# mohammadasim98/mv-ldm

Hardware: AMD Instinct MI355X
Metric: denoised views/sec @ 256x256, 4 views, 50 DDIM steps (higher is better)
Workload: dtype bf16

## Files before the change

### mv_ldm_amd/_lib.py

```python
from __future__ import annotations

import ctypes as C
from pathlib import Path

LIB_PATH = Path(__file__).resolve().parent / "csrc" / "libmvldm_hip.so"

ABI_VERSION = 7
F32, BF16, F16 = 0, 1, 2
EPI_NONE, EPI_SILU, EPI_GEGLU, EPI_GELU = 0, 1, 2, 3
RAYS_RAW, RAYS_POSITIONAL, RAYS_SRT = 0, 1, 2
ELT_COPY, ELT_SILU, ELT_GELU = 0, 1, 2
NORM_BWD_STORE = 0x100
GN_MAX_CHUNKS = 32

(OP_IGEMM, OP_GROUPNORM, OP_LAYERNORM, OP_ATTENTION, OP_TIMESTEP_EMBED, OP_ELTWISE, OP_DDIM_STEP, OP_DDIM_ADVANCE,
 OP_NCHW_TO_NHWC, OP_NHWC_TO_NCHW, OP_MEMCPY, OP_RAY_ENCODE, OP_POSTERIOR_SAMPLE,
 OP_WGRAD, OP_ATTENTION_BWD, OP_GROUPNORM_BWD, OP_LAYERNORM_BWD, OP_COLSUM, OP_TRAIN_ELTWISE, OP_POOL2X2, OP_ZERO_INSERT,
 OP_ADD_NOISE, OP_MSE_LOSS, OP_FILL_ZERO, OP_PAR_BEGIN, OP_PAR_NEXT, OP_PAR_END, OP_GATHER_ROWS, OP_ATTN_MERGE) = range(1, 30)
TE_SILU_BWD, TE_ADD, TE_GEGLU_FWD, TE_GEGLU_BWD, TE_GELU_BWD = 0, 1, 2, 3, 4

vp, i32, f32, sz = C.c_void_p, C.c_int32, C.c_float, C.c_size_t


class IgemmDesc(C.Structure):
    _fields_ = [("src0", vp), ("src1", vp), ("weight", vp), ("bias", vp), ("row_bias", vp), ("residual", vp),
                ("dst", vp), ("workspace", vp),
                ("c0", i32), ("c1", i32),
                ("n_img", i32), ("h_in", i32), ("w_in", i32), ("h_out", i32), ("w_out", i32),
                ("ksize", i32), ("stride", i32), ("pad", i32), ("upsample", i32),
                ("n_out", i32), ("n_pad", i32), ("k_pad", i32),
                ("row_bias_ld", i32), ("epilogue", i32), ("act_dtype", i32), ("dst_dtype", i32),
                ("splitk", i32), ("tile", i32), ("k_order", i32), ("dst_ld", i32), ("out_scale", f32), ("workspace_bytes", sz)]


class _GroupNorm(C.Structure):
    _fields_ = [("x", vp), ("x1", vp), ("y", vp), ("gamma", vp), ("beta", vp), ("stats_ws", vp),
                ("n_img", i32), ("hw", i32), ("c0", i32), ("c1", i32), ("groups", i32), ("silu", i32), ("dtype", i32),
                ("eps", f32), ("stats_out", vp)]


class _LayerNorm(C.Structure):
    _fields_ = [("x", vp), ("y", vp), ("gamma", vp), ("beta", vp), ("rows", i32), ("c", i32), ("dtype", i32), ("eps", f32)]


class _Attention(C.Structure):
    _fields_ = [("q", vp), ("k", vp), ("v", vp), ("out", vp), ("seg", vp),
                ("ld_q", i32), ("ld_k", i32), ("ld_v", i32), ("ld_o", i32), ("heads", i32), ("head_dim", i32),
                ("n_seg", i32), ("max_q_len", i32), ("dtype", i32), ("scale", f32), ("lse", vp), ("lse_ld", i32)]


class _Temb(C.Structure):
    _fields_ = [("timesteps", vp), ("freqs", vp), ("out", vp), ("n", i32), ("dim", i32), ("flip", i32), ("dst_dtype", i32)]


class _Eltwise(C.Structure):
    _fields_ = [("x", vp), ("y", vp), ("n", sz), ("op", i32), ("src_dtype", i32), ("dst_dtype", i32)]


class _Ddim(C.Structure):
    _fields_ = [("eps", vp), ("x_t", vp), ("x_next", vp), ("cond_img", vp), ("uncond_img", vp), ("coef", vp),
                ("step_ptr", vp), ("unet_in", vp),
                ("n_tgt", i32), ("hw", i32), ("c", i32), ("unet_in_c", i32), ("unet_in_dtype", i32), ("cfg_scale", f32),
                ("n_steps", i32), ("clip_range", f32)]


class _Advance(C.Structure):
    _fields_ = [("step_ptr", vp), ("t_table", vp), ("timesteps", vp), ("tgt_rows", vp), ("n_steps", i32), ("n_rows", i32)]


class _Layout(C.Structure):
    _fields_ = [("src", vp), ("dst", vp), ("n_img", i32), ("c", i32), ("hw", i32), ("other_c", i32),
                ("other_c_off", i32), ("dtype", i32), ("clamp01", i32), ("scale", f32), ("shift", f32), ("img_map", vp)]


class _Rays(C.Structure):
    _fields_ = [("extrinsics", vp), ("intrinsics", vp), ("out_nchw", vp), ("out_nhwc", vp), ("img_map", vp),
                ("n_cam", i32), ("h", i32), ("w", i32), ("nhwc_c", i32), ("nhwc_c_off", i32), ("nhwc_dtype", i32),
                ("mode", i32), ("n_origin_octaves", i32), ("n_dir_octaves", i32), ("plucker", i32)]


class _Posterior(C.Structure):
    _fields_ = [("moments", vp), ("noise", vp), ("out", vp), ("n", i32), ("c", i32), ("hw", i32), ("scale", f32)]


class _Memcpy(C.Structure):
    _fields_ = [("src", vp), ("dst", vp), ("bytes", sz)]


class _AttnMerge(C.Structure):
    _fields_ = [("oa", vp), ("ob", vp), ("out", vp), ("lse_a", vp), ("lse_b", vp), ("a_img", vp), ("b_img", vp), ("out_img", vp),
                ("n_img", i32), ("tokens", i32), ("heads", i32), ("head_dim", i32), ("ld_a", i32), ("ld_b", i32), ("ld_o", i32),
                ("lse_ld_a", i32), ("lse_ld_b", i32), ("dtype", i32)]


class _Gather(C.Structure):
    _fields_ = [("src", vp), ("dst", vp), ("src_index", vp), ("dst_index", vp), ("row_bytes", sz), ("n_rows", i32)]


class PackJob(C.Structure):
    _fields_ = [("src", vp), ("dst", vp), ("n_out", i32), ("c_in", i32), ("ksize", i32), ("c_pad", i32), ("n_pad", i32), ("k_pad", i32),
                ("geglu", i32), ("k_order", i32), ("transpose", i32), ("c_off", i32), ("n_rows", i32), ("kind", i32), ("blocks", i32),
                ("block0", i32)]


class WgradDesc(C.Structure):
    _fields_ = [("src0", vp), ("src1", vp), ("dy", vp), ("grad", vp), ("workspace", vp), ("workspace_bytes", sz),
                ("c0", i32), ("c1", i32), ("c_in", i32),
                ("n_img", i32), ("h_in", i32), ("w_in", i32), ("h_out", i32), ("w_out", i32),
                ("ksize", i32), ("stride", i32), ("pad", i32), ("upsample", i32),
                ("n_out", i32), ("dy_ld", i32), ("act_dtype", i32), ("accumulate", i32)]


class AttnBwdDesc(C.Structure):
    _fields_ = [("q", vp), ("k", vp), ("v", vp), ("out", vp), ("dout", vp), ("dq", vp), ("dk", vp), ("dv", vp),
                ("lse", vp), ("delta", vp), ("seg", vp),
                ("ld_q", i32), ("ld_k", i32), ("ld_v", i32), ("ld_o", i32), ("ld_do", i32), ("ld_dq", i32), ("ld_dk", i32), ("ld_dv", i32),
                ("heads", i32), ("head_dim", i32), ("n_seg", i32), ("max_q_len", i32), ("max_kv_len", i32), ("total_q_rows", i32),
                ("stat_ld", i32), ("dtype", i32), ("scale", f32)]


class _GroupNormBwd(C.Structure):
    _fields_ = [("x0", vp), ("x1", vp), ("dy", vp), ("dx0", vp), ("dx1", vp), ("gamma", vp), ("beta", vp), ("stats", vp),
                ("dgamma", vp), ("dbeta", vp), ("workspace", vp), ("workspace_bytes", sz),
                ("n_img", i32), ("hw", i32), ("c0", i32), ("c1", i32), ("groups", i32), ("silu", i32), ("dtype", i32)]


class _LayerNormBwd(C.Structure):
    _fields_ = [("x", vp), ("dy", vp), ("dx", vp), ("gamma", vp), ("dgamma", vp), ("dbeta", vp), ("workspace", vp),
                ("workspace_bytes", sz), ("rows", i32), ("c", i32), ("dtype", i32), ("eps", f32)]


class _Colsum(C.Structure):
    _fields_ = [("x", vp), ("dst", vp), ("workspace", vp), ("workspace_bytes", sz),
                ("n_seg", i32), ("rows_per_seg", i32), ("n", i32), ("ld", i32), ("ld_dst", i32), ("per_seg", i32),
                ("accumulate", i32), ("dtype", i32)]


class _TrainEltwise(C.Structure):
    _fields_ = [("a", vp), ("b", vp), ("out", vp), ("rows", sz), ("op", i32), ("d", i32), ("a_dtype", i32), ("dtype", i32)]


class _Resample(C.Structure):
    _fields_ = [("src", vp), ("dst", vp), ("n_img", i32), ("h", i32), ("w", i32), ("c", i32), ("dtype", i32)]


class _AddNoise(C.Structure):
    _fields_ = [("x0", vp), ("noise", vp), ("coef", vp), ("dst", vp), ("img_map", vp),
                ("n", i32), ("c", i32), ("hw", i32), ("dst_c", i32), ("dst_c_off", i32), ("dst_dtype", i32)]


class _Mse(C.Structure):
    _fields_ = [("pred", vp), ("noise", vp), ("tgt_img", vp), ("loss", vp), ("dpred", vp), ("workspace", vp),
                ("n_tgt", i32), ("hw", i32), ("c", i32), ("accumulate", i32), ("dpred_c", i32), ("dpred_dtype", i32),
                ("loss_scale", f32), ("grad_scale", f32), ("amp_scale", vp)]


class AmpState(C.Structure):
    _fields_ = [("scale", f32), ("growth_tracker", i32), ("adam_step", i32), ("found_inf", i32), ("skipped", i32), ("reserved", i32 * 3)]


class _Fill(C.Structure):
    _fields_ = [("dst", vp), ("bytes", sz)]


class _OpUnion(C.Union):
    _fields_ = [("igemm", IgemmDesc), ("groupnorm", _GroupNorm), ("layernorm", _LayerNorm), ("attention", _Attention),
                ("temb", _Temb), ("eltwise", _Eltwise), ("ddim", _Ddim), ("advance", _Advance), ("layout", _Layout),
                ("memcpy_", _Memcpy), ("gather", _Gather), ("attn_merge", _AttnMerge), ("rays", _Rays), ("posterior", _Posterior),
                ("wgrad", WgradDesc), ("attention_bwd", AttnBwdDesc), ("groupnorm_bwd", _GroupNormBwd),
                ("layernorm_bwd", _LayerNormBwd), ("colsum", _Colsum), ("train_eltwise", _TrainEltwise), ("resample", _Resample),
                ("add_noise", _AddNoise), ("mse", _Mse), ("fill", _Fill)]


class Op(C.Structure):
    _fields_ = [("kind", i32), ("tag", i32), ("u", _OpUnion)]


SIGNATURES = {
    "mvldm_abi_version": (C.c_int, []),
    "mvldm_build_flags": (C.c_int, []),
    "mvldm_last_error": (C.c_char_p, []),
    "mvldm_device_info": (C.c_int, [C.POINTER(C.c_int), C.POINTER(sz), C.c_char_p, C.c_int]),
    "mvldm_igemm_fwd": (C.c_int, [C.POINTER(IgemmDesc), vp]),
    "mvldm_igemm_workspace_bytes": (sz, [C.POINTER(IgemmDesc)]),
    "mvldm_pack_weight": (C.c_int, [vp, vp] + [C.c_int] * 12 + [vp]),
    "mvldm_pack_skinny": (C.c_int, [vp, vp, C.c_int, C.c_int, C.c_int, C.c_int, vp]),
    "mvldm_igemm_skinny_config": (C.c_int, [C.POINTER(IgemmDesc)]),
    "mvldm_pack_job_prepare": (C.c_int, [C.POINTER(PackJob), C.c_int]),
    "mvldm_pack_weight_batch": (C.c_int, [vp, C.c_int, vp, C.c_int, C.c_int, vp]),
    "mvldm_groupnorm_fwd": (C.c_int, [vp, vp, vp, vp, vp, C.c_int, C.c_int, C.c_int, C.c_int, C.c_int, f32, C.c_int, C.c_int, vp, vp, vp]),
    "mvldm_groupnorm_passes": (C.c_int, [C.c_int] * 5),
    "mvldm_layernorm_fwd": (C.c_int, [vp, vp, vp, vp, C.c_int, C.c_int, f32, C.c_int, vp]),
    "mvldm_attention_fwd": (C.c_int, [vp, vp, vp, vp] + [C.c_int] * 6 + [vp, C.c_int, C.c_int, f32, C.c_int, vp, C.c_int, vp]),
    "mvldm_igemm_wgrad": (C.c_int, [C.POINTER(WgradDesc), vp]),
    "mvldm_colsum": (C.c_int, [vp, vp, vp, sz] + [C.c_int] * 8 + [vp]),
    "mvldm_groupnorm_bwd": (C.c_int, [vp] * 10 + [C.c_int] * 7 + [vp, sz, vp]),
    "mvldm_layernorm_bwd": (C.c_int, [vp] * 6 + [C.c_int, C.c_int, f32, C.c_int, vp, sz, vp]),
    "mvldm_attention_bwd": (C.c_int, [C.POINTER(AttnBwdDesc), vp]),
    "mvldm_train_eltwise": (C.c_int, [C.c_int, vp, vp, vp, sz, C.c_int, C.c_int, C.c_int, vp]),
    "mvldm_pool2x2_sum": (C.c_int, [vp, vp] + [C.c_int] * 5 + [vp]),
    "mvldm_zero_insert2x": (C.c_int, [vp, vp] + [C.c_int] * 5 + [vp]),
    "mvldm_add_noise": (C.c_int, [vp, vp, vp, vp] + [C.c_int] * 6 + [vp, vp]),
    "mvldm_mse_loss": (C.c_int, [vp, vp, vp, C.c_int, C.c_int, C.c_int, vp, C.c_int, f32, vp, C.c_int, C.c_int, f32, vp, vp]),
    "mvldm_grad_norm": (C.c_int, [vp, sz, vp, f32, vp, vp, vp]),
    "mvldm_adamw_step": (C.c_int, [vp, vp, vp, vp, sz, f32, f32, f32, f32, f32, C.c_int, f32, vp, vp]),
    "mvldm_mse_loss_amp": (C.c_int, [vp, vp, vp, C.c_int, C.c_int, C.c_int, vp, C.c_int, f32, vp, C.c_int, C.c_int, f32, vp, vp, vp]),
    "mvldm_grad_norm_amp": (C.c_int, [vp, sz, vp, f32, vp, vp, vp, vp]),
    "mvldm_adamw_step_amp": (C.c_int, [vp, vp, vp, vp, sz, f32, f32, f32, f32, f32, f32, vp, vp, vp]),
    "mvldm_amp_update": (C.c_int, [vp, f32, f32, C.c_int, vp]),
    "mvldm_timestep_embed_fwd": (C.c_int, [vp, vp, vp, C.c_int, C.c_int, C.c_int, C.c_int, vp]),
    "mvldm_eltwise_fwd": (C.c_int, [vp, vp, sz, C.c_int, C.c_int, C.c_int, vp]),
    "mvldm_ddim_cfg_step": (C.c_int, [vp, vp, vp, vp, vp, C.c_int, C.c_int, C.c_int, f32, vp, vp, vp, C.c_int, C.c_int, C.c_int, f32, vp]),
    "mvldm_ddim_advance": (C.c_int, [vp, vp, C.c_int, vp, vp, C.c_int, vp]),
    "mvldm_gather_rows": (C.c_int, [vp, vp, vp, vp, C.c_int, sz, vp]),
    "mvldm_attention_merge": (C.c_int, [vp] * 8 + [C.c_int] * 10 + [vp]),
    "mvldm_ddpm_cfg_step": (C.c_int, [vp, vp, vp, vp, vp, sz, f32, vp, f32, vp]),
    "mvldm_ema_update": (C.c_int, [vp, vp, sz, f32, vp]),
    "mvldm_image_metrics_workspace_bytes": (sz, [C.c_int] * 4),
    "mvldm_image_metrics": (C.c_int, [vp, vp] + [C.c_int] * 5 + [vp, vp, vp, sz, vp]),
    "mvldm_lpips_workspace_bytes": (sz, [C.c_int] * 3),
    "mvldm_lpips_tap_slots": (C.c_int, [C.c_int] * 3),
    "mvldm_lpips_prep": (C.c_int, [vp, vp, vp] + [C.c_int] * 6 + [vp]),
    "mvldm_lpips_relu": (C.c_int, [vp, sz, C.c_int, vp]),
    "mvldm_lpips_tap": (C.c_int, [vp, vp, vp] + [C.c_int] * 5 + [vp, sz, C.c_int, C.c_int, vp]),
    "mvldm_lpips_fold": (C.c_int, [vp, sz, C.c_int, C.c_int, C.c_int, vp, vp]),
    "mvldm_dists_workspace_bytes": (sz, [C.c_int] * 3),
    "mvldm_dists_stat_slots": (C.c_int, [C.c_int] * 3),
    "mvldm_dists_prep": (C.c_int, [vp, vp, vp] + [C.c_int] * 5 + [vp]),
    "mvldm_dists_stats": (C.c_int, [vp, vp] + [C.c_int] * 5 + [vp, sz, C.c_int, C.c_int, vp]),
    "mvldm_dists_l2pool": (C.c_int, [vp, vp] + [C.c_int] * 5 + [vp]),
    "mvldm_dists_fold": (C.c_int, [vp, sz, C.c_int, C.c_int, C.c_int, vp, vp, vp, vp]),
    "mvldm_fid_workspace_bytes": (sz, [C.c_int] * 4),
    "mvldm_fid_pool_slots": (C.c_int, [C.c_int] * 3),
    "mvldm_fid_prep": (C.c_int, [vp, C.c_int, vp] + [C.c_int] * 7 + [vp]),
    "mvldm_fid_pool": (C.c_int, [vp] + [C.c_int] * 5 + [vp, sz, vp]),
    "mvldm_fid_accumulate": (C.c_int, [vp, sz] + [C.c_int] * 4 + [vp, vp, vp]),
    "mvldm_fid_compute": (C.c_int, [vp, vp, C.c_int, vp, vp, vp]),
    "mvldm_inception_workspace_bytes": (sz, [C.c_int] * 3),
    "mvldm_inception_prep": (C.c_int, [vp, C.c_int, vp] + [C.c_int] * 7 + [vp, sz, vp]),
    "mvldm_inception_unfold": (C.c_int, [vp, vp] + [C.c_int] * 9 + [vp]),
    "mvldm_inception_maxpool": (C.c_int, [vp, vp] + [C.c_int] * 9 + [vp]),
    "mvldm_inception_avgpool": (C.c_int, [vp, vp] + [C.c_int] * 7 + [vp]),
    "mvldm_inception_concat": (C.c_int, [vp, vp, sz] + [C.c_int] * 5 + [vp]),
    "mvldm_inception_features": (C.c_int, [vp] + [C.c_int] * 5 + [vp, vp]),
    "mvldm_frechet_accumulate": (C.c_int, [vp, C.c_int, C.c_int, vp, vp]),
    "mvldm_frechet_workspace_bytes": (sz, [C.c_int]),
    "mvldm_frechet_compute": (C.c_int, [vp, vp, C.c_int, vp, sz, vp, vp, vp]),
    "mvldm_kid_workspace_bytes": (sz, [C.c_int, C.c_int]),
    "mvldm_kid_compute": (C.c_int, [vp, C.c_int, vp, C.c_int, C.c_int, vp, vp, C.c_int, C.c_int, vp, sz, vp, vp, vp, vp]),
    "mvldm_crop_shim_workspace_bytes": (sz, [C.c_int] * 5),
    "mvldm_crop_shim": (C.c_int, [vp, C.c_int, vp] + [C.c_int] * 5 + [vp, sz, C.POINTER(C.c_int), vp]),
    "mvldm_crop_shim_axis": (C.c_int, [C.c_int] * 4 + [C.POINTER(i32), C.POINTER(i32), C.c_int]),
    "mvldm_nchw_to_nhwc": (C.c_int, [vp, vp] + [C.c_int] * 6 + [f32, f32, vp, vp]),
    "mvldm_ray_channels": (C.c_int, [C.c_int, C.c_int, C.c_int]),
    "mvldm_ray_encode": (C.c_int, [vp, vp, C.c_int, C.c_int, C.c_int, vp, vp, C.c_int, C.c_int, C.c_int, vp] + [C.c_int] * 4 + [vp]),
    "mvldm_posterior_sample": (C.c_int, [vp, vp, vp, C.c_int, C.c_int, C.c_int, f32, vp]),
    "mvldm_nhwc_to_nchw": (C.c_int, [vp, vp] + [C.c_int] * 6 + [f32, f32, C.c_int, vp]),
    "mvldm_op_run": (C.c_int, [C.POINTER(Op), vp]),
    "mvldm_plan_create": (C.c_int, [C.POINTER(Op), C.c_int, C.POINTER(vp)]),
    "mvldm_plan_num_ops": (C.c_int, [vp]),
    "mvldm_plan_run": (C.c_int, [vp, vp]),
    "mvldm_plan_run_range": (C.c_int, [vp, C.c_int, C.c_int, vp]),
    "mvldm_plan_capture": (C.c_int, [vp, vp]),
    "mvldm_plan_replay": (C.c_int, [vp, vp]),
    "mvldm_plan_profile": (C.c_int, [vp, vp, C.c_int, C.POINTER(f32)]),
    "mvldm_plan_destroy": (None, [vp]),
}

_lib = None


class MvldmError(RuntimeError):
    pass


_EXPERIMENT_KNOBS = ("MVLDM_ADAMW_NT", "MVLDM_ATTN_QB", "MVLDM_ATTN_WIDE_VALU", "MVLDM_GN_NTHR", "MVLDM_GN_SPAN", "MVLDM_GN_TWOPASS", "MVLDM_GN_WIDE",
                     "MVLDM_IGEMM_FAKE", "MVLDM_IGEMM_GROUP", "MVLDM_IGEMM_NOSTAGE", "MVLDM_IGEMM_PX", "MVLDM_IGEMM_SYNC", "MVLDM_IGEMM_TARGET",
                     "MVLDM_LPP_CPT", "MVLDM_LPP_FAKE", "MVLDM_PLAN_SERIAL", "MVLDM_PW_FAKE", "MVLDM_PW_GM", "MVLDM_PW_TN", "MVLDM_RS_FAKE", "MVLDM_SK_FAKE",
                     "MVLDM_STREAM_STORES", "MVLDM_WGRAD_DIRECT", "MVLDM_WGRAD_TARGET", "MVLDM_WGRAD_WIDE", "MVLDM_WGRAD_WIDE_BP",
                     "MVLDM_WGRAD_WIDE_TARGET", "MVLDM_WGRAD_XCD", "MVLDM_WS_FAKE")


def load(required: bool = True):
    global _lib
    if _lib is not None:
        return _lib
    if not LIB_PATH.exists():
        if required:
            raise MvldmError(f"{LIB_PATH} is missing: run `python -c 'import __graft_entry__ as g; g.build()'` "
                             "(there is no CPU / PyTorch fallback for the HIP path)")
        return None
    lib = C.CDLL(str(LIB_PATH))
    for name, (res, args) in SIGNATURES.items():
        fn = getattr(lib, name)
        fn.restype, fn.argtypes = res, args
    if lib.mvldm_abi_version() != ABI_VERSION:
        raise MvldmError("libmvldm_hip.so ABI version mismatch")
    if not (lib.mvldm_build_flags() & 1) and "_exp" not in LIB_PATH.name:
        import os
        stale = sorted(k for k in _EXPERIMENT_KNOBS if k in os.environ)
        if stale:
            raise MvldmError(f"{', '.join(stale)} set, but {LIB_PATH.name} was built without -DMVLDM_EXPERIMENTS and ignores it: build an "
                             "experiment library (MVLDM_EXPERIMENTS=1 python -m mv_ldm_amd._build --force, or tools/*_probe.sh + --lib) or unset it")
    _lib = lib
    return lib


def check(rc: int):
    if rc != 0:
        raise MvldmError(f"mvldm error {rc}: {load().mvldm_last_error().decode()}")
```

### mv_ldm_amd/csrc/norm.hip

```cpp
#include "common.h"
#include <algorithm>
#include <cstdlib>

namespace mvldm {

template <typename T>
__global__ __launch_bounds__(256) void gn_stats_kernel(const T* __restrict__ x0, const T* __restrict__ x1, int c0,
                                                       double* __restrict__ partial, int hw, int c, int groups,
                                                       int rows_per_chunk, int nchunk) {
    constexpr int EPC = Elt<T>::EPC;
    __shared__ double s_sum[64], s_sq[64];
    const int img = blockIdx.x / nchunk, chunk = blockIdx.x % nchunk;
    const int ncc = c / EPC;
    const int cpg = c / groups;
    const int tid = threadIdx.x;
    if (tid < 64) { s_sum[tid] = 0.0; s_sq[tid] = 0.0; }
    __syncthreads();
    const int r_begin = chunk * rows_per_chunk, r_end = min(hw, r_begin + rows_per_chunk);
    const int nthr = blockDim.x;
    for (int cc0 = 0; cc0 < ncc; cc0 += nthr) {
        const int span = min(ncc - cc0, nthr);
        const int R = max(1, nthr / span);
        const int cc = cc0 + tid % span, rl = tid / span;
        double s[EPC], q[EPC];
#pragma unroll
        for (int i = 0; i < EPC; ++i) { s[i] = 0.0; q[i] = 0.0; }
        if (rl < R) {
            const int ch0 = cc * EPC;
            const bool first = ch0 < c0;
            const int cs = first ? c0 : c - c0;
            const T* base = (first ? x0 + ch0 : x1 + (ch0 - c0)) + ((size_t)img * hw) * cs;
            for (int r = r_begin + rl; r < r_end; r += R) {
                const Chunk<T> v = load_chunk<T>(base + (size_t)r * cs);
#pragma unroll
                for (int i = 0; i < EPC; ++i) {
                    const double f = (double)v.get(i);
                    s[i] += f;
                    q[i] += f * f;
                }
            }
#pragma unroll
            for (int i = 0; i < EPC; ++i) {
                const int g = (cc * EPC + i) / cpg;
                atomicAdd(&s_sum[g], s[i]);
                atomicAdd(&s_sq[g], q[i]);
            }
        }
    }
    __syncthreads();
    if (tid < groups) {
        double* o = partial + (((size_t)img * nchunk + chunk) * groups + tid) * 2;
        o[0] = s_sum[tid];
        o[1] = s_sq[tid];
    }
}

template <typename T>
__global__ __launch_bounds__(256) void gn_apply_kernel(const T* __restrict__ x0, const T* __restrict__ x1, int c0,
                                                       T* __restrict__ y,
                                                       const float* __restrict__ gamma, const float* __restrict__ beta,
                                                       const double* __restrict__ partial, int hw, int c, int groups,
                                                       int rows_per_chunk, int nchunk, float eps, int silu, float* __restrict__ stats_out) {
    constexpr int EPC = Elt<T>::EPC;
    extern __shared__ __attribute__((aligned(16))) char smem_raw[];
    float* s_scale = reinterpret_cast<float*>(smem_raw);
    float* s_shift = s_scale + c;
    float* s_mean = s_shift + c;
    float* s_rstd = s_mean + groups;
    const int img = blockIdx.x / nchunk, chunk = blockIdx.x % nchunk;
    const int tid = threadIdx.x;
    const int cpg = c / groups;
    if (tid < groups) {
        double s = 0.0, q = 0.0;
        for (int k = 0; k < nchunk; ++k) {
            const double* pp = partial + (((size_t)img * nchunk + k) * groups + tid) * 2;
            s += pp[0];
            q += pp[1];
        }
        const double n = (double)hw * cpg;
        const double mean = s / n;
        double var = q / n - mean * mean;
        var = var > 0.0 ? var : 0.0;
        s_mean[tid] = (float)mean;
        s_rstd[tid] = (float)(1.0 / sqrt(var + (double)eps));
        if (stats_out && chunk == 0) {
            stats_out[((size_t)img * groups + tid) * 2] = s_mean[tid];
            stats_out[((size_t)img * groups + tid) * 2 + 1] = s_rstd[tid];
        }
    }
    __syncthreads();
    for (int ch = tid; ch < c; ch += blockDim.x) {
        const int g = ch / cpg;
        const float sc = s_rstd[g] * gamma[ch];
        s_scale[ch] = sc;
        s_shift[ch] = beta[ch] - s_mean[g] * sc;
    }
    __syncthreads();
    const int ncc = c / EPC;
    const int r_begin = chunk * rows_per_chunk, r_end = min(hw, r_begin + rows_per_chunk);
    const size_t total = (size_t)(r_end - r_begin) * ncc;
    const size_t row0 = (size_t)img * hw + r_begin;
    T* yb = y + row0 * c;
    const int c1 = c - c0;
    (void)total;
    const int nthr = blockDim.x;
    for (int cc0 = 0; cc0 < ncc; cc0 += nthr) {
        const int span = min(ncc - cc0, nthr);
        const int R = max(1, nthr / span);
        const int cc = cc0 + tid % span, rl = tid / span;
        if (rl >= R) continue;
        const int ch0 = cc * EPC;
        float sc[EPC], sh[EPC];
#pragma unroll
        for (int i = 0; i < EPC; ++i) { sc[i] = s_scale[ch0 + i]; sh[i] = s_shift[ch0 + i]; }
        const bool first = ch0 < c0;
        const int cs = first ? c0 : c1;
        const T* src = (first ? x0 + ch0 : x1 + (ch0 - c0)) + row0 * cs;
        T* dst = yb + ch0;
        const int nrows = r_end - r_begin;
        for (int r = rl; r < nrows; r += R) {
            const Chunk<T> v = load_chunk<T>(src + (size_t)r * cs);
            Chunk<T> o;
#pragma unroll
            for (int i = 0; i < EPC; ++i) {
                float f = fmaf(v.get(i), sc[i], sh[i]);
                if (silu) f = f * __builtin_amdgcn_rcpf(1.0f + __builtin_amdgcn_exp2f(-1.4426950408889634f * f));
                o.set(i, f);
            }
            store_chunk<T>(dst + (size_t)r * c, o);
        }
    }
}

template <typename T, int KT>
__global__ __launch_bounds__(1024) void gn_fused_kernel(const T* __restrict__ x0, const T* __restrict__ x1, int c0,
                                                        T* __restrict__ y, const float* __restrict__ gamma,
                                                        const float* __restrict__ beta, int hw, int c, int groups, int span,
                                                        float eps, int silu, float* __restrict__ stats_out) {
    constexpr int EPC = Elt<T>::EPC;
    __shared__ double s_sum[64], s_sq[64];
    __shared__ float s_mean[64], s_rstd[64];
    const int bid = xcd_remap(blockIdx.x, gridDim.x);
    const int nspan = c / span, img = bid / nspan, sp = bid - img * nspan;
    const int cps = span / EPC, cpg = c / groups;
    const int tid = threadIdx.x, nthr = blockDim.x;
    const int ch = tid % cps, row0 = tid / cps, rstep = nthr / cps;
    const int col = sp * span + ch * EPC;
    const bool first = col < c0;
    const int cs = first ? c0 : c - c0;
    const T* src = (first ? x0 + col : x1 + (col - c0)) + (size_t)img * hw * cs;
    const int gbase = (sp * span) / cpg, ng = span / cpg;
    const int g0 = col / cpg - gbase;
    const int split = min(EPC, (gbase + g0 + 1) * cpg - col);
    if (tid < 64) { s_sum[tid] = 0.0; s_sq[tid] = 0.0; }
    __syncthreads();
    Chunk<T> v[KT];
    float s[EPC], q[EPC];
#pragma unroll
    for (int i = 0; i < EPC; ++i) { s[i] = 0.f; q[i] = 0.f; }
#pragma unroll
    for (int k = 0; k < KT; ++k) {
        const int row = row0 + k * rstep;
        if (row < hw) {
            v[k] = load_chunk<T>(src + (size_t)row * cs);
#pragma unroll
            for (int i = 0; i < EPC; ++i) {
                const float f = v[k].get(i);
                s[i] += f;
                q[i] = fmaf(f, f, q[i]);
            }
        }
    }
    double sa = 0.0, qa = 0.0, sb = 0.0, qb = 0.0;
#pragma unroll
    for (int i = 0; i < EPC; ++i) {
        if (i < split) { sa += (double)s[i]; qa += (double)q[i]; }
        else { sb += (double)s[i]; qb += (double)q[i]; }
    }
    atomicAdd(&s_sum[g0], sa);
    atomicAdd(&s_sq[g0], qa);
    if (split < EPC) {
        atomicAdd(&s_sum[g0 + 1], sb);
        atomicAdd(&s_sq[g0 + 1], qb);
    }
    __syncthreads();
    if (tid < ng) {
        const double n = (double)hw * cpg;
        const double mean = s_sum[tid] / n;
        double var = s_sq[tid] / n - mean * mean;
        var = var > 0.0 ? var : 0.0;
        s_mean[tid] = (float)mean;
        s_rstd[tid] = (float)(1.0 / sqrt(var + (double)eps));
        if (stats_out) {
            stats_out[((size_t)img * groups + gbase + tid) * 2] = s_mean[tid];
            stats_out[((size_t)img * groups + gbase + tid) * 2 + 1] = s_rstd[tid];
        }
    }
    __syncthreads();
    float sc[EPC], sh[EPC];
#pragma unroll
    for (int i = 0; i < EPC; ++i) {
        const int g = i < split ? g0 : g0 + 1;
        sc[i] = s_rstd[g] * gamma[col + i];
        sh[i] = beta[col + i] - s_mean[g] * sc[i];
    }
    T* dst = y + (size_t)img * hw * c + col;
#pragma unroll
    for (int k = 0; k < KT; ++k) {
        const int row = row0 + k * rstep;
        if (row < hw) {
            Chunk<T> o;
#pragma unroll
            for (int i = 0; i < EPC; ++i) {
                float f = fmaf(v[k].get(i), sc[i], sh[i]);
                if (silu) f = f * __builtin_amdgcn_rcpf(1.0f + __builtin_amdgcn_exp2f(-1.4426950408889634f * f));
                o.set(i, f);
            }
            store_chunk<T>(dst + (size_t)row * c, o);
        }
    }
}

static int gn_fused_plan(int hw, int c, int groups, int epc, int n_img, int& nthr, int& kt) {
    static const int force_wide = knob_int("MVLDM_GN_WIDE", 0);
    const int cpg = c / groups;
    if (!((cpg >= epc && true) || (epc % cpg == 0 && epc / cpg == 2))) return 0;
    auto gcd = [](int a, int b) { while (b) { int t = a % b; a = b; b = t; } return a; };
    const int base = cpg / gcd(cpg, epc) * epc;
    if (base > c || c % base) return 0;
    int best = 0;
    static const int x_span = knob_int("MVLDM_GN_SPAN", 0), x_nthr = knob_int("MVLDM_GN_NTHR", 1024);
    for (int m = 1; base * m <= c; ++m) {
        const int span = base * m;
        if (c % span || span / cpg > 64) continue;
        if (x_span && x_span <= c && span != x_span) continue;
        const int cps = span / epc;
        const int l = cps / gcd(cps, 64) * 64;
        if (l > 1024) continue;
        int n = std::max(l, std::min(1024, x_nthr) / l * l);
        const long long chunks = (long long)hw * cps;
        while (n > l && (long long)(n - l) >= chunks) n -= l;
        const int k = (int)((chunks + n - 1) / n);
        if (k > 16) continue;
        const bool enough = (long long)n_img * (c / span) >= 512;
        if (best == 0 || force_wide || enough) { best = span; nthr = n; kt = k; }
        if (!force_wide && !enough) break;
    }
    return best;
}

template <typename T, int MAXCH>
__global__ __launch_bounds__(256) void layernorm_kernel(const T* __restrict__ x, T* __restrict__ y,
                                                        const float* __restrict__ gamma, const float* __restrict__ beta,
                                                        int rows, int c, float eps) {
    constexpr int EPC = Elt<T>::EPC;
    const int lane = threadIdx.x & 63;
    const int row = blockIdx.x * (blockDim.x >> 6) + (threadIdx.x >> 6);
    if (row >= rows) return;
    const int ncc = c / EPC;
    const T* xr = x + (size_t)row * c;
    Chunk<T> v[MAXCH];
    float s = 0.f;
#pragma unroll
    for (int k = 0; k < MAXCH; ++k) {
        const int cc = lane + k * 64;
        if (cc < ncc) {
            v[k] = load_chunk<T>(xr + cc * EPC);
#pragma unroll
            for (int i = 0; i < EPC; ++i) s += v[k].get(i);
        }
    }
    const float mean = wave_sum(s) / (float)c;
    float q = 0.f;
#pragma unroll
    for (int k = 0; k < MAXCH; ++k) {
        const int cc = lane + k * 64;
        if (cc < ncc) {
#pragma unroll
            for (int i = 0; i < EPC; ++i) {
                const float d = v[k].get(i) - mean;
                q += d * d;
            }
        }
    }
    const float rstd = rsqrtf(wave_sum(q) / (float)c + eps);
    T* yr = y + (size_t)row * c;
#pragma unroll
    for (int k = 0; k < MAXCH; ++k) {
        const int cc = lane + k * 64;
        if (cc < ncc) {
            Chunk<T> o;
#pragma unroll
            for (int i = 0; i < EPC; ++i) {
                const int ch = cc * EPC + i;
                o.set(i, (v[k].get(i) - mean) * rstd * gamma[ch] + beta[ch]);
            }
            store_chunk<T>(yr + cc * EPC, o);
        }
    }
}

template <typename T, int LPR, int CPL>
__global__ __launch_bounds__(256) void layernorm_rows_kernel(const T* __restrict__ x, T* __restrict__ y, const float* __restrict__ gamma,
                                                             const float* __restrict__ beta, int rows, int c, float eps) {
    constexpr int EPC = Elt<T>::EPC, RPW = 64 / LPR;
    const int lane = threadIdx.x & 63, sub = lane & (LPR - 1), rsel = lane / LPR;
    float g[CPL][EPC], b[CPL][EPC];
#pragma unroll
    for (int k = 0; k < CPL; ++k)
#pragma unroll
        for (int i = 0; i < EPC; ++i) {
            g[k][i] = gamma[(sub + k * LPR) * EPC + i];
            b[k][i] = beta[(sub + k * LPR) * EPC + i];
        }
    const float inv_c = 1.0f / (float)c;
    const int stride = gridDim.x * 4 * RPW;
    for (int row0 = (blockIdx.x * 4 + (threadIdx.x >> 6)) * RPW; row0 < rows; row0 += stride) {
        const int row = row0 + rsel;
        const bool ok = row < rows;
        const T* xr = x + (size_t)(ok ? row : 0) * c;
        Chunk<T> v[CPL];
#pragma unroll
        for (int k = 0; k < CPL; ++k) v[k] = load_chunk<T>(xr + (sub + k * LPR) * EPC);
        float s = 0.f;
#pragma unroll
        for (int k = 0; k < CPL; ++k)
#pragma unroll
            for (int i = 0; i < EPC; ++i) s += v[k].get(i);
#pragma unroll
        for (int o = LPR / 2; o > 0; o >>= 1) s += __shfl_xor(s, o, 64);
        const float mean = s * inv_c;
        float q = 0.f;
#pragma unroll
        for (int k = 0; k < CPL; ++k)
#pragma unroll
            for (int i = 0; i < EPC; ++i) {
                const float d = v[k].get(i) - mean;
                q += d * d;
            }
#pragma unroll
        for (int o = LPR / 2; o > 0; o >>= 1) q += __shfl_xor(q, o, 64);
        const float rstd = rsqrtf(q * inv_c + eps);
        if (!ok) continue;
        T* yr = y + (size_t)row * c;
#pragma unroll
        for (int k = 0; k < CPL; ++k) {
            Chunk<T> o;
#pragma unroll
            for (int i = 0; i < EPC; ++i) o.set(i, (v[k].get(i) - mean) * rstd * g[k][i] + b[k][i]);
            store_chunk<T>(yr + (sub + k * LPR) * EPC, o);
        }
    }
}

template <typename T, int CPL>
static bool layernorm_rows_launch(const T* x, T* y, const float* gamma, const float* beta, int rows, int c, float eps, int lpr, hipStream_t s) {
    const int rpw = 64 / lpr;
    const int blocks = std::min((rows + 4 * rpw - 1) / (4 * rpw), 256 * 16);
    if (lpr == 8) hipLaunchKernelGGL((layernorm_rows_kernel<T, 8, CPL>), dim3(blocks), dim3(256), 0, s, x, y, gamma, beta, rows, c, eps);
    else if (lpr == 16) hipLaunchKernelGGL((layernorm_rows_kernel<T, 16, CPL>), dim3(blocks), dim3(256), 0, s, x, y, gamma, beta, rows, c, eps);
    else if (lpr == 32) hipLaunchKernelGGL((layernorm_rows_kernel<T, 32, CPL>), dim3(blocks), dim3(256), 0, s, x, y, gamma, beta, rows, c, eps);
    else return false;
    return true;
}

int groupnorm_run(const void* x, const void* x1, void* y, const float* gamma, const float* beta, int n_img, int hw, int c0,
                  int c1, int groups, float eps, int silu, int dtype, void* stats_ws, float* stats_out, hipStream_t s) {
    MVLDM_REQUIRE(groups > 0 && groups <= 64 && (c0 + c1) % groups == 0, "groupnorm: c=%d groups=%d", c0 + c1, groups);
    if (n_img == 0 || hw == 0) return MVLDM_OK;
    MVLDM_REQUIRE(x && y && gamma && beta && stats_ws, "groupnorm: null pointer");
    MVLDM_REQUIRE((c1 == 0) == (x1 == nullptr), "groupnorm: x1/c1 mismatch");
    const int c = c0 + c1;
    MVLDM_REQUIRE(groups > 0 && groups <= 64 && c % groups == 0, "groupnorm: c=%d groups=%d", c, groups);
    const int epc = dtype == MVLDM_F32 ? 4 : 8;
    MVLDM_REQUIRE(c0 % epc == 0 && c1 % epc == 0, "groupnorm: channels (%d,%d) must be multiples of %d", c0, c1, epc);
    if (n_img == 0 || hw == 0) return MVLDM_OK;
    static const int no_fused = knob_int("MVLDM_GN_TWOPASS", 0);
    int f_nthr = 0, f_kt = 0;
    const int f_span = no_fused ? 0 : gn_fused_plan(hw, c, groups, epc, n_img, f_nthr, f_kt);
    if (f_span) {
        return dispatch_dtype(dtype, [&](auto t) {
            using T = decltype(t);
            const dim3 grid(n_img * (c / f_span)), block(f_nthr);
#define MVLDM_GN_FUSED(KT_)                                                                                             \
    hipLaunchKernelGGL((gn_fused_kernel<T, KT_>), grid, block, 0, s, reinterpret_cast<const T*>(x), reinterpret_cast<const T*>(x1), \
                       c0, reinterpret_cast<T*>(y), gamma, beta, hw, c, groups, f_span, eps, silu, stats_out)
            if (f_kt <= 2) MVLDM_GN_FUSED(2);
            else if (f_kt <= 4) MVLDM_GN_FUSED(4);
            else if (f_kt <= 8) MVLDM_GN_FUSED(8);
            else if (f_kt <= 12) MVLDM_GN_FUSED(12);
            else MVLDM_GN_FUSED(16);
#undef MVLDM_GN_FUSED
            return check_launch();
        });
    }
    int nchunk = std::min(MVLDM_GN_MAX_CHUNKS, std::max(1, std::min(hw / 8, (1024 + n_img - 1) / n_img)));
    const int rows_per_chunk = (hw + nchunk - 1) / nchunk;
    nchunk = (hw + rows_per_chunk - 1) / rows_per_chunk;
    const size_t smem = (size_t)(2 * c + 2 * groups) * sizeof(float);
    return dispatch_dtype(dtype, [&](auto t) {
        using T = decltype(t);
        hipLaunchKernelGGL(gn_stats_kernel<T>, dim3(n_img * nchunk), dim3(256), 0, s, reinterpret_cast<const T*>(x),
                           reinterpret_cast<const T*>(x1), c0, reinterpret_cast<double*>(stats_ws), hw, c, groups,
                           rows_per_chunk, nchunk);
        int rc = check_launch();
        if (rc) return rc;
        hipLaunchKernelGGL(gn_apply_kernel<T>, dim3(n_img * nchunk), dim3(256), smem, s, reinterpret_cast<const T*>(x),
                           reinterpret_cast<const T*>(x1), c0, reinterpret_cast<T*>(y), gamma, beta, reinterpret_cast<const double*>(stats_ws), hw, c, groups,
                           rows_per_chunk, nchunk, eps, silu, stats_out);
        return check_launch();
    });
}

int layernorm_run(const void* x, void* y, const float* gamma, const float* beta, int rows, int c, float eps, int dtype,
                  hipStream_t s) {
    if (rows == 0) return MVLDM_OK;
    MVLDM_REQUIRE(x && y && gamma && beta, "layernorm: null pointer");
    const int epc = dtype == MVLDM_F32 ? 4 : 8;
    MVLDM_REQUIRE(c % epc == 0, "layernorm: c=%d must be a multiple of %d", c, epc);
    const int ncc = c / epc;
    MVLDM_REQUIRE(ncc <= 64 * 16, "layernorm: c=%d too wide", c);
    if (rows == 0) return MVLDM_OK;
    const int blocks = (rows + 3) / 4;
    return dispatch_dtype(dtype, [&](auto t) {
        using T = decltype(t);
        const T* xp = reinterpret_cast<const T*>(x);
        T* yp = reinterpret_cast<T*>(y);
        if constexpr (sizeof(T) == 2) {
            if (rows >= 1024) {
                for (int cpl = 5; cpl >= 3; --cpl) {
                    if (ncc % cpl) continue;
                    const int lpr = ncc / cpl;
                    if (lpr != 8 && lpr != 16 && lpr != 32) continue;
                    const bool ok = cpl == 5 ? layernorm_rows_launch<T, 5>(xp, yp, gamma, beta, rows, c, eps, lpr, s)
                                  : cpl == 4 ? layernorm_rows_launch<T, 4>(xp, yp, gamma, beta, rows, c, eps, lpr, s)
                                             : layernorm_rows_launch<T, 3>(xp, yp, gamma, beta, rows, c, eps, lpr, s);
                    if (ok) return check_launch();
                }
            }
        }
        if (ncc <= 64) hipLaunchKernelGGL((layernorm_kernel<T, 1>), dim3(blocks), dim3(256), 0, s, xp, yp, gamma, beta, rows, c, eps);
        else if (ncc <= 128) hipLaunchKernelGGL((layernorm_kernel<T, 2>), dim3(blocks), dim3(256), 0, s, xp, yp, gamma, beta, rows, c, eps);
        else if (ncc <= 256) hipLaunchKernelGGL((layernorm_kernel<T, 4>), dim3(blocks), dim3(256), 0, s, xp, yp, gamma, beta, rows, c, eps);
        else if (ncc <= 512) hipLaunchKernelGGL((layernorm_kernel<T, 8>), dim3(blocks), dim3(256), 0, s, xp, yp, gamma, beta, rows, c, eps);
        else hipLaunchKernelGGL((layernorm_kernel<T, 16>), dim3(blocks), dim3(256), 0, s, xp, yp, gamma, beta, rows, c, eps);
        return check_launch();
    });
}

}

extern "C" int mvldm_groupnorm_passes(int n_img, int hw, int c, int groups, int dtype) {
    if (n_img <= 0 || hw <= 0 || groups <= 0 || c <= 0 || c % groups) return 3;
    static const int no_fused = mvldm::knob_int("MVLDM_GN_TWOPASS", 0);
    int nthr = 0, kt = 0;
    return (!no_fused && mvldm::gn_fused_plan(hw, c, groups, dtype == MVLDM_F32 ? 4 : 8, n_img, nthr, kt)) ? 2 : 3;
}

extern "C" int mvldm_groupnorm_fwd(const void* x0, const void* x1, void* y, const float* gamma, const float* beta,
                                   int n_img, int hw, int c0, int c1, int groups, float eps, int silu, int dtype,
                                   void* stats_ws, float* stats_out, mvldm_stream_t stream) {
    return mvldm::groupnorm_run(x0, x1, y, gamma, beta, n_img, hw, c0, c1, groups, eps, silu, dtype, stats_ws, stats_out,
                                (hipStream_t)stream);
}

extern "C" int mvldm_layernorm_fwd(const void* x, void* y, const float* gamma, const float* beta, int rows, int c,
                                   float eps, int dtype, mvldm_stream_t stream) {
    return mvldm::layernorm_run(x, y, gamma, beta, rows, c, eps, dtype, (hipStream_t)stream);
}
```

Measured before the change: 49.90.

## Add register-resident fused GroupNorm kernel with LDS spill for tail chunks

Adds a new one-pass GroupNorm kernel that keeps each thread's input chunks in registers (with up to two extra chunks parked in LDS), reduces per-group statistics through shared memory, then applies the affine and optional SiLU from the held values without re-reading global memory. A new planner sizes thread counts by rows times chunks-per-span, and the kernel uses packed float2 math for the accumulation and epilogue. It is the default path (MVLDM_GN_FORM=1), with the old fused kernel kept behind the knob. The aim is to remove the second global read and cut the reduction overhead, at the cost of higher register pressure and more template instances.

```diff
diff --git a/mv_ldm_amd/_lib.py b/mv_ldm_amd/_lib.py
--- a/mv_ldm_amd/_lib.py
+++ b/mv_ldm_amd/_lib.py
@@ -274,7 +274,7 @@
     pass
 
 
-_EXPERIMENT_KNOBS = ("MVLDM_ADAMW_NT", "MVLDM_ATTN_QB", "MVLDM_ATTN_WIDE_VALU", "MVLDM_GN_NTHR", "MVLDM_GN_SPAN", "MVLDM_GN_TWOPASS", "MVLDM_GN_WIDE",
+_EXPERIMENT_KNOBS = ("MVLDM_ADAMW_NT", "MVLDM_ATTN_QB", "MVLDM_ATTN_WIDE_VALU", "MVLDM_GN_FORM", "MVLDM_GN_NTHR", "MVLDM_GN_SPAN", "MVLDM_GN_TWOPASS", "MVLDM_GN_WIDE",
                      "MVLDM_IGEMM_FAKE", "MVLDM_IGEMM_GROUP", "MVLDM_IGEMM_NOSTAGE", "MVLDM_IGEMM_PX", "MVLDM_IGEMM_SYNC", "MVLDM_IGEMM_TARGET",
                      "MVLDM_LPP_CPT", "MVLDM_LPP_FAKE", "MVLDM_PLAN_SERIAL", "MVLDM_PW_FAKE", "MVLDM_PW_GM", "MVLDM_PW_TN", "MVLDM_RS_FAKE", "MVLDM_SK_FAKE",
                      "MVLDM_STREAM_STORES", "MVLDM_WGRAD_DIRECT", "MVLDM_WGRAD_TARGET", "MVLDM_WGRAD_WIDE", "MVLDM_WGRAD_WIDE_BP",
diff --git a/mv_ldm_amd/csrc/norm.hip b/mv_ldm_amd/csrc/norm.hip
--- a/mv_ldm_amd/csrc/norm.hip
+++ b/mv_ldm_amd/csrc/norm.hip
@@ -221,7 +221,7 @@
     }
 }
 
-static int gn_fused_plan(int hw, int c, int groups, int epc, int n_img, int& nthr, int& kt) {
+static int gn_fused_plan_v0(int hw, int c, int groups, int epc, int n_img, int& nthr, int& kt) {
     static const int force_wide = knob_int("MVLDM_GN_WIDE", 0);
     const int cpg = c / groups;
     if (!((cpg >= epc && true) || (epc % cpg == 0 && epc / cpg == 2))) return 0;
@@ -249,6 +249,221 @@
     return best;
 }
 
+constexpr int GN_RES_THREADS = 512, GN_RES_KR = 20, GN_RES_KL = 2;
+constexpr int GN_ONE_THREADS = 1024, GN_ONE_KT = 16;
+
+typedef float gn_f32x2 __attribute__((ext_vector_type(2)));
+
+template <typename T>
+__device__ __forceinline__ void gn_fold(const Chunk<T>& v, gn_f32x2 (&s)[Elt<T>::EPC / 2], gn_f32x2 (&q)[Elt<T>::EPC / 2]) {
+#pragma unroll
+    for (int i = 0; i < Elt<T>::EPC / 2; ++i) {
+        const gn_f32x2 f = {v.get(2 * i), v.get(2 * i + 1)};
+        s[i] += f;
+        q[i] = __builtin_elementwise_fma(f, f, q[i]);
+    }
+}
+
+template <typename T, bool SILU>
+__device__ __forceinline__ Chunk<T> gn_affine(const Chunk<T>& v, const gn_f32x2 (&sc)[Elt<T>::EPC / 2], const gn_f32x2 (&sh)[Elt<T>::EPC / 2]) {
+    Chunk<T> o;
+#pragma unroll
+    for (int i = 0; i < Elt<T>::EPC / 2; ++i) {
+        gn_f32x2 f = __builtin_elementwise_fma(gn_f32x2{v.get(2 * i), v.get(2 * i + 1)}, sc[i], sh[i]);
+        if (SILU) {
+            const gn_f32x2 a = f * -1.4426950408889634f;
+            const gn_f32x2 d = gn_f32x2{__builtin_amdgcn_exp2f(a.x), __builtin_amdgcn_exp2f(a.y)} + 1.0f;
+            f = f * gn_f32x2{__builtin_amdgcn_rcpf(d.x), __builtin_amdgcn_rcpf(d.y)};
+        }
+        o.set(2 * i, f.x);
+        o.set(2 * i + 1, f.y);
+    }
+    return o;
+}
+
+template <typename T, int KR, int KL, bool SILU>
+__global__ __launch_bounds__(GN_ONE_THREADS) void gn_resident_kernel(const T* __restrict__ x0, const T* __restrict__ x1, int c0,
+                                                                        T* __restrict__ y, const float* __restrict__ gamma,
+                                                                        const float* __restrict__ beta, int hw, int c, int groups,
+                                                                        int span, int nact, float eps,
+                                                                        float* __restrict__ stats_out) {
+    constexpr int EPC = Elt<T>::EPC;
+    constexpr int KA = KR - KL;
+    static_assert(KL <= KR, "the LDS-bound chunks borrow registers of the later register chunks");
+    extern __shared__ __attribute__((aligned(16))) char gn_smem[];
+    __shared__ float s_mean[64], s_rstd[64];
+    const int bid = xcd_remap(blockIdx.x, gridDim.x);
+    const int nspan = c / span, img = bid / nspan, sp = bid - img * nspan;
+    const int cps = span / EPC, cpg = c / groups;
+    const int tid = threadIdx.x;
+    const bool active = tid < nact;
+    const int ch = tid % cps, rstep = nact / cps;
+    const int row0 = active ? tid / cps : 0;
+    const int col = sp * span + ch * EPC;
+    const bool first = col < c0;
+    const int cs = first ? c0 : c - c0;
+    const T* src = (first ? x0 + col : x1 + (col - c0)) + (size_t)img * hw * cs;
+    const int gbase = (sp * span) / cpg, ng = span / cpg;
+    const int g0 = col / cpg - gbase;
+    const int split = min(EPC, (gbase + g0 + 1) * cpg - col);
+    double* slot = reinterpret_cast<double*>(gn_smem);
+    u32x4* held = reinterpret_cast<u32x4*>(gn_smem + (size_t)nact * 32) + tid;
+
+    constexpr int TAIL = 2;
+    auto fetch = [&](int j) {
+        const int row = row0 + j * rstep;
+        Chunk<T> r = load_chunk<T>(src + (size_t)(j >= KR + KL - TAIL ? min(row, hw - 1) : row) * cs);
+        if (j >= KR + KL - TAIL && row >= hw) r.zero();
+        return r;
+    };
+    Chunk<T> v[KR], t[KL > 0 ? KL : 1];
+#pragma unroll
+    for (int k = 0; k < KL; ++k) t[k] = fetch(KR + k);
+#pragma unroll
+    for (int k = 0; k < KA; ++k) v[k] = fetch(k);
+    gn_f32x2 s[EPC / 2], q[EPC / 2];
+#pragma unroll
+    for (int i = 0; i < EPC / 2; ++i) { s[i] = gn_f32x2{0.f, 0.f}; q[i] = gn_f32x2{0.f, 0.f}; }
+#pragma unroll
+    for (int k = 0; k < KL; ++k) {
+        gn_fold<T>(t[k], s, q);
+        if (active && row0 + (KR + k) * rstep < hw) held[k * nact] = t[k].raw;
+    }
+#pragma unroll
+    for (int k = KA; k < KR; ++k) v[k] = fetch(k);
+#pragma unroll
+    for (int k = 0; k < KR; ++k) gn_fold<T>(v[k], s, q);
+
+    double sa = 0.0, qa = 0.0, sb = 0.0, qb = 0.0;
+#pragma unroll
+    for (int i = 0; i < EPC; ++i) {
+        if (i < split) { sa += (double)s[i / 2][i % 2]; qa += (double)q[i / 2][i % 2]; }
+        else { sb += (double)s[i / 2][i % 2]; qb += (double)q[i / 2][i % 2]; }
+    }
+    if (active) {
+        slot[tid] = sa;
+        slot[nact + tid] = qa;
+        slot[2 * nact + tid] = sb;
+        slot[3 * nact + tid] = qb;
+    }
+    __syncthreads();
+    {
+        const int nthr = blockDim.x;
+        int ts = 64;
+        while (ts > 1 && ts * ng > nthr) ts >>= 1;
+        const int team = tid / ts, l = tid & (ts - 1), nteam = nthr / ts;
+        for (int gi = 0; gi < ng; gi += nteam) {
+            const int g = gi + team;
+            double a = 0.0, b = 0.0;
+            if (g < ng) {
+                const int lo = g * cpg;
+                const int c_lo = lo / EPC, nc = (lo + cpg - 1) / EPC - c_lo + 1, cnt = rstep * nc;
+                for (int j = l; j < cnt; j += ts) {
+                    const int r = j / nc, ci = c_lo + (j - r * nc);
+                    const int o = (ci * EPC >= lo ? 0 : 2 * nact) + r * cps + ci;
+                    a += slot[o];
+                    b += slot[o + nact];
+                }
+            }
+#pragma unroll
+            for (int o = 32; o > 0; o >>= 1) {
+                if (o < ts) {
+                    a += __shfl_xor(a, o, 64);
+                    b += __shfl_xor(b, o, 64);
+                }
+            }
+            if (g < ng && l == 0) {
+                const double n = (double)hw * cpg;
+                const double mean = a / n;
+                double var = b / n - mean * mean;
+                var = var > 0.0 ? var : 0.0;
+                const float mf = (float)mean, rf = (float)(1.0 / sqrt(var + (double)eps));
+                s_mean[g] = mf;
+                s_rstd[g] = rf;
+                if (stats_out) {
+                    stats_out[((size_t)img * groups + gbase + g) * 2] = mf;
+                    stats_out[((size_t)img * groups + gbase + g) * 2 + 1] = rf;
+                }
+            }
+        }
+    }
+    __syncthreads();
+    gn_f32x2 sc[EPC / 2], sh[EPC / 2];
+#pragma unroll
+    for (int i = 0; i < EPC; ++i) {
+        const int g = i < split ? g0 : g0 + 1;
+        const float m = s_rstd[g] * gamma[col + i];
+        sc[i / 2][i % 2] = m;
+        sh[i / 2][i % 2] = beta[col + i] - s_mean[g] * m;
+    }
+    T* dst = y + (size_t)img * hw * c + col;
+#pragma unroll
+    for (int k = 0; k < KR; ++k) asm volatile("" : "+v"(v[k].raw));
+    int row0s = row0;
+    asm volatile("" : "+v"(row0s));
+#pragma unroll
+    for (int k = 0; k < KR; ++k) {
+        const int row = row0s + k * rstep;
+        if (active && row < hw) store_chunk<T>(dst + (size_t)row * c, gn_affine<T, SILU>(v[k], sc, sh));
+    }
+#pragma unroll
+    for (int k = 0; k < KL; ++k) {
+        const int row = row0s + (KR + k) * rstep;
+        if (active && row < hw) {
+            Chunk<T> h;
+            h.raw = held[k * nact];
+            store_chunk<T>(dst + (size_t)row * c, gn_affine<T, SILU>(h, sc, sh));
+        }
+    }
+}
+
+static int gn_fused_plan(int hw, int c, int groups, int epc, int n_img, int& nthr, int& kt) {
+    static const int force_wide = knob_int("MVLDM_GN_WIDE", 0);
+    static const int x_span = knob_int("MVLDM_GN_SPAN", 0), x_nthr = std::min(GN_ONE_THREADS, knob_int("MVLDM_GN_NTHR", 0));
+    const int cpg = c / groups;
+    if (!(cpg >= epc || (epc % cpg == 0 && epc / cpg == 2))) return 0;
+    auto gcd = [](int a, int b) { while (b) { int t = a % b; a = b; b = t; } return a; };
+    const int base = cpg / gcd(cpg, epc) * epc;
+    if (base > c || c % base) return 0;
+    int best = 0;
+    for (int m = 1; base * m <= c; ++m) {
+        const int span = base * m;
+        if (c % span || span / cpg > 64) continue;
+        if (x_span && x_span <= c && span != x_span) continue;
+        const int cps = span / epc;
+        int rows = 0, k = 0;
+        for (int cap : {x_nthr ? x_nthr : GN_RES_THREADS, x_nthr ? 0 : GN_ONE_THREADS}) {
+            if (cap < cps) continue;
+            const int r = std::min(hw, cap / cps), kk = (hw + r - 1) / r;
+            if (kk > (cap > GN_RES_THREADS ? GN_ONE_KT : GN_RES_KR + GN_RES_KL)) continue;
+            rows = r;
+            k = kk;
+            break;
+        }
+        if (!rows) continue;
+        const bool enough = (long long)n_img * (c / span) >= 512;
+        if (best == 0 || force_wide || enough) { best = span; nthr = rows * cps; kt = k; }
+        if (!force_wide && !enough) break;
+    }
+    return best;
+}
+
+static int gn_form() {
+    static const int form = knob_int("MVLDM_GN_FORM", 1);
+    return form;
+}
+
+template <typename T, int KR, int KL, bool SILU>
+static int gn_resident_launch(const void* x, const void* x1, int c0, void* y, const float* gamma, const float* beta, int n_img, int hw,
+                              int c, int groups, int span, int nact, int kt, float eps, float* stats_out, hipStream_t s) {
+    auto kern = gn_resident_kernel<T, KR, KL, SILU>;
+    static_assert(GN_ONE_THREADS * 32 <= 48 * 1024 && GN_RES_THREADS * (32 + 16 * GN_RES_KL) <= 48 * 1024, "dynamic LDS within the default limit");
+    const int smem = nact * (32 + 16 * std::max(0, kt - KR));
+    hipLaunchKernelGGL(kern, dim3(n_img * (c / span)), dim3((nact + 63) / 64 * 64), smem, s, reinterpret_cast<const T*>(x),
+                       reinterpret_cast<const T*>(x1), c0, reinterpret_cast<T*>(y), gamma, beta, hw, c, groups, span, nact, eps, stats_out);
+    return check_launch();
+}
+
 template <typename T, int MAXCH>
 __global__ __launch_bounds__(256) void layernorm_kernel(const T* __restrict__ x, T* __restrict__ y,
                                                         const float* __restrict__ gamma, const float* __restrict__ beta,
@@ -366,18 +581,43 @@
 
 int groupnorm_run(const void* x, const void* x1, void* y, const float* gamma, const float* beta, int n_img, int hw, int c0,
                   int c1, int groups, float eps, int silu, int dtype, void* stats_ws, float* stats_out, hipStream_t s) {
-    MVLDM_REQUIRE(groups > 0 && groups <= 64 && (c0 + c1) % groups == 0, "groupnorm: c=%d groups=%d", c0 + c1, groups);
+    const int c = c0 + c1;
+    MVLDM_REQUIRE(groups > 0 && groups <= 64 && c % groups == 0, "groupnorm: c=%d groups=%d", c, groups);
     if (n_img == 0 || hw == 0) return MVLDM_OK;
     MVLDM_REQUIRE(x && y && gamma && beta && stats_ws, "groupnorm: null pointer");
     MVLDM_REQUIRE((c1 == 0) == (x1 == nullptr), "groupnorm: x1/c1 mismatch");
-    const int c = c0 + c1;
-    MVLDM_REQUIRE(groups > 0 && groups <= 64 && c % groups == 0, "groupnorm: c=%d groups=%d", c, groups);
     const int epc = dtype == MVLDM_F32 ? 4 : 8;
     MVLDM_REQUIRE(c0 % epc == 0 && c1 % epc == 0, "groupnorm: channels (%d,%d) must be multiples of %d", c0, c1, epc);
-    if (n_img == 0 || hw == 0) return MVLDM_OK;
     static const int no_fused = knob_int("MVLDM_GN_TWOPASS", 0);
     int f_nthr = 0, f_kt = 0;
-    const int f_span = no_fused ? 0 : gn_fused_plan(hw, c, groups, epc, n_img, f_nthr, f_kt);
+    if (!no_fused && gn_form() != 0) {
+        const int r_span = gn_fused_plan(hw, c, groups, epc, n_img, f_nthr, f_kt);
+        if (r_span) {
+            return dispatch_dtype(dtype, [&](auto t) {
+                using T = decltype(t);
+#define MVLDM_GN_RES(KR_, KL_)                                                                                                              \
+    (silu ? gn_resident_launch<T, KR_, KL_, true>(x, x1, c0, y, gamma, beta, n_img, hw, c, groups, r_span, f_nthr, f_kt, eps, stats_out, s)   \
+          : gn_resident_launch<T, KR_, KL_, false>(x, x1, c0, y, gamma, beta, n_img, hw, c, groups, r_span, f_nthr, f_kt, eps, stats_out, s))
+                static_assert(GN_RES_KR == 20 && GN_RES_KL == 2, "instances below");
+                switch (f_kt <= 1 ? 0 : (f_kt + 1) / 2) {
+                    case 0: return MVLDM_GN_RES(1, 0);
+                    case 1: return MVLDM_GN_RES(2, 0);
+                    case 2: return MVLDM_GN_RES(4, 0);
+                    case 3: return MVLDM_GN_RES(6, 0);
+                    case 4: return MVLDM_GN_RES(8, 0);
+                    case 5: return MVLDM_GN_RES(10, 0);
+                    case 6: return MVLDM_GN_RES(12, 0);
+                    case 7: return MVLDM_GN_RES(14, 0);
+                    case 8: return MVLDM_GN_RES(16, 0);
+                    case 9: return MVLDM_GN_RES(18, 0);
+                    case 10: return MVLDM_GN_RES(20, 0);
+                    default: return MVLDM_GN_RES(20, 2);
+                }
+#undef MVLDM_GN_RES
+            });
+        }
+    }
+    const int f_span = (no_fused || gn_form() != 0) ? 0 : gn_fused_plan_v0(hw, c, groups, epc, n_img, f_nthr, f_kt);
     if (f_span) {
         return dispatch_dtype(dtype, [&](auto t) {
             using T = decltype(t);
@@ -454,7 +694,10 @@
     if (n_img <= 0 || hw <= 0 || groups <= 0 || c <= 0 || c % groups) return 3;
     static const int no_fused = mvldm::knob_int("MVLDM_GN_TWOPASS", 0);
     int nthr = 0, kt = 0;
-    return (!no_fused && mvldm::gn_fused_plan(hw, c, groups, dtype == MVLDM_F32 ? 4 : 8, n_img, nthr, kt)) ? 2 : 3;
+    const int epc = dtype == MVLDM_F32 ? 4 : 8;
+    const int span = no_fused ? 0 : mvldm::gn_form() != 0 ? mvldm::gn_fused_plan(hw, c, groups, epc, n_img, nthr, kt)
+                                                           : mvldm::gn_fused_plan_v0(hw, c, groups, epc, n_img, nthr, kt);
+    return span ? 2 : 3;
 }
 
 extern "C" int mvldm_groupnorm_fwd(const void* x0, const void* x1, void* y, const float* gamma, const float* beta,
```

After: 50.12, median of 6. No clear change (+0.5%).
